# taintpro98/rnd-semantic-segmentation

Hardware: AMD Instinct MI355X
Metric: train images/sec at 769x769 bf16 (DeepLabV2-ResNet101 + ASPP) (higher is better)
Workload: dtype bf16; 1 GPU; train_src.py DeepLabV2-R101 bf16, 769x769 synthetic Cityscapes crops, batch 8 per GPU, 1xMI355X; global_batch=8, parallelism=dp1, weights=formula (synthetic), hip_graph_replay=False

## Files before the change

### rnd_semantic_segmentation_amd/csrc/igemm_common.h

```cpp
#pragma once
#include "mi_common.h"

namespace {

__device__ __attribute__((aligned(256))) uint32_t g_zero_page[64];

struct IgemmParams {
    const __bf16* A;
    const __bf16* Wp;
    void* out;
    const float* scale;
    const float* bias;
    const __bf16* res;
    const __bf16* msk;
    uint16_t* mask_out;
    int M, N, Ca, T;
    int Ho, Wo, Ha, Wa;
    int ksz, stride, pad, dil, mode;
    int flags, zgw;
    float alpha;
    int m_tiles, n_tiles;
    int korder;
    float* stats;
    const float* pilot;
};

__device__ __forceinline__ float igemm_row16_sum(float v) {
    v += __builtin_bit_cast(float, __builtin_amdgcn_update_dpp(0, __builtin_bit_cast(int, v), 0xB1, 0xF, 0xF, true));
    v += __builtin_bit_cast(float, __builtin_amdgcn_update_dpp(0, __builtin_bit_cast(int, v), 0x4E, 0xF, 0xF, true));
    v += __builtin_bit_cast(float, __builtin_amdgcn_update_dpp(0, __builtin_bit_cast(int, v), 0x141, 0xF, 0xF, true));
    v += __builtin_bit_cast(float, __builtin_amdgcn_update_dpp(0, __builtin_bit_cast(int, v), 0x140, 0xF, 0xF, true));
    return v;
}

__device__ __forceinline__ void glds16(const char* gsrc, char* lds_wave_base) {
    __builtin_amdgcn_global_load_lds((const __attribute__((address_space(1))) void*)gsrc,
                                     (__attribute__((address_space(3))) void*)lds_wave_base, 16, 0, 0);
}
__device__ __forceinline__ void glds16_nt(const char* gsrc, char* lds_wave_base) {
    __builtin_amdgcn_global_load_lds((const __attribute__((address_space(1))) void*)gsrc,
                                     (__attribute__((address_space(3))) void*)lds_wave_base, 16, 0, 2);
}

__device__ __forceinline__ void blds16(__amdgpu_buffer_rsrc_t rsrc, unsigned voffset, unsigned soffset, char* lds_wave_base) {
    __builtin_amdgcn_raw_ptr_buffer_load_lds(rsrc, (__attribute__((address_space(3))) void*)lds_wave_base, 16, voffset, soffset, 0, 0);
}


template <int MT, int EPI, bool WANT_RES = true>
__device__ __forceinline__ void igemm_fetch_epilogue(const IgemmParams& p, int m0, int n0, int wm, int wn, int frow, int fq, bf16x8 (&pres)[MT][2],
                                                     unsigned (&pbits)[MT], const int* mrow = nullptr) {
    const int flags = (EPI >= 0 ? EPI : p.flags) & (WANT_RES ? ~0 : ~MI_EPI_RESIDUAL);
    const int nbp = n0 + wn * 64 + 8 * fq;
#pragma unroll
    for (int j = 0; j < MT; ++j) {
        const int m = mrow ? (mrow[j] < 0 ? p.M : mrow[j]) : m0 + wm * (MT * 16) + j * 16 + frow;
        const long o0 = (long)(m < p.M ? m : 0) * p.N + (nbp < p.N ? nbp : 0);
        const long o1 = (long)(m < p.M ? m : 0) * p.N + (nbp + 32 < p.N ? nbp + 32 : 0);
        if (flags & MI_EPI_RESIDUAL) {
            pres[j][0] = *reinterpret_cast<const bf16x8*>(p.res + o0);
            pres[j][1] = *reinterpret_cast<const bf16x8*>(p.res + o1);
        }
        if (flags & MI_EPI_BITMASK) {
            const uint8_t* mb = reinterpret_cast<const uint8_t*>(p.msk);
            pbits[j] = (unsigned)mb[o0 >> 3] | ((unsigned)mb[o1 >> 3] << 8);
        }
    }
}

template <int MT, int EPI, bool STAGED = false>
__device__ __forceinline__ void igemm_epilogue(const IgemmParams& p, f32x4 (&acc)[4][MT], int m0, int n0, int wm, int wn, int frow, int fq,
                                               bf16x8 (&pres)[MT][2], unsigned (&pbits)[MT], char* stage = nullptr, bool mask_lds = false,
                                               const int* mrow = nullptr) {
    const int flags = EPI >= 0 ? EPI : p.flags;
    constexpr bool STATS = EPI >= 0 && (EPI & MI_EPI_STATS) != 0;
    float st0[STATS ? 16 : 1], st1[STATS ? 16 : 1];
    const int nb = n0 + wn * 64 + 8 * fq;
    f32x4 esc[4], ebi[4];
    if (flags & MI_EPI_SCALE_BIAS) {
#pragma unroll
        for (int i = 0; i < 4; ++i) {
            const int ni = nb + 32 * (i >> 1) + 4 * (i & 1);
            const int n = (ni < p.N) ? ni : 0;
            esc[i] = *reinterpret_cast<const f32x4*>(p.scale + n);
            ebi[i] = *reinterpret_cast<const f32x4*>(p.bias + n);
        }
    }
    f32x4 epil[4];
    if constexpr (STATS) {
#pragma unroll
        for (int i = 0; i < 4; ++i) {
            const int ni = nb + 32 * (i >> 1) + 4 * (i & 1);
            epil[i] = *reinterpret_cast<const f32x4*>(p.pilot + ((ni < p.N) ? ni : 0));
        }
#pragma unroll
        for (int k = 0; k < 16; ++k) st0[k] = st1[k] = 0.f;
#pragma unroll
        for (int i = 0; i < 4; ++i) asm volatile("" ::"v"(epil[i]));
    }
    if (flags & MI_EPI_SCALE_BIAS) {
#pragma unroll
        for (int i = 0; i < 4; ++i) asm volatile("" ::"v"(esc[i]), "v"(ebi[i]));
    }
    if (flags & MI_EPI_RESIDUAL) {
#pragma unroll
        for (int j = 0; j < MT; ++j) asm volatile("" ::"v"(pres[j][0]), "v"(pres[j][1]));
    }
    if (flags & MI_EPI_BITMASK) {
#pragma unroll
        for (int j = 0; j < MT; ++j) asm volatile("" ::"v"(pbits[j]));
    }
#pragma unroll
    for (int j = 0; j < MT; ++j) {
        const int m = mrow ? (mrow[j] < 0 ? p.M : mrow[j]) : m0 + wm * (MT * 16) + j * 16 + frow;
        if (m >= p.M) continue;
        const long o = (long)m * p.N + nb;
        f32x4 v[4];
#pragma unroll
        for (int i = 0; i < 4; ++i) v[i] = acc[i][j];
        if (flags & MI_EPI_SCALE_BIAS) {
#pragma unroll
            for (int i = 0; i < 4; ++i) v[i] = v[i] * esc[i] + ebi[i];
        }
        if (flags & MI_EPI_RESIDUAL) {
#pragma unroll
            for (int h = 0; h < 2; ++h) {
                if (nb + 32 * h < p.N) {
                    const bf16x8 r = pres[j][h];
#pragma unroll
                    for (int e = 0; e < 8; ++e) v[2 * h + (e >> 2)][e & 3] += (float)r[e];
                }
            }
        }
        if (flags & MI_EPI_RELU) {
            if (flags & MI_EPI_LEAKY) {
#pragma unroll
                for (int i = 0; i < 4; ++i)
#pragma unroll
                    for (int e = 0; e < 4; ++e) v[i][e] = v[i][e] > 0.f ? v[i][e] : p.alpha * v[i][e];
            } else {
#pragma unroll
                for (int i = 0; i < 4; ++i)
#pragma unroll
                    for (int e = 0; e < 4; ++e) asm("v_max_f32 %0, 0, %1" : "=v"(v[i][e]) : "v"(v[i][e]));
            }
        }
        if (flags & MI_EPI_MASK) {
#pragma unroll
            for (int h = 0; h < 2; ++h) {
                if (nb + 32 * h < p.N) {
                    const bf16x8 k = *reinterpret_cast<const bf16x8*>(p.msk + o + 32 * h);
#pragma unroll
                    for (int e = 0; e < 8; ++e)
                        v[2 * h + (e >> 2)][e & 3] = ((float)k[e] > 0.f) ? v[2 * h + (e >> 2)][e & 3] : 0.f;
                }
            }
        }
        if (flags & MI_EPI_BITMASK) {
            const float neg = (flags & MI_EPI_LEAKY) ? p.alpha : 0.f;
#pragma unroll
            for (int h = 0; h < 2; ++h) {
                if (nb + 32 * h < p.N) {
                    const unsigned bits = (pbits[j] >> (8 * h)) & 0xffu;
                    if (flags & MI_EPI_LEAKY) {
#pragma unroll
                        for (int c = 0; c < 8; ++c) v[2 * h + (c >> 2)][c & 3] = ((bits >> c) & 1u) ? v[2 * h + (c >> 2)][c & 3] : neg * v[2 * h + (c >> 2)][c & 3];
                    } else {
#pragma unroll
                        for (int c = 0; c < 8; ++c) {
                            const unsigned keep = (unsigned)__builtin_amdgcn_sbfe((int)bits, c, 1);
                            v[2 * h + (c >> 2)][c & 3] = __uint_as_float(__float_as_uint(v[2 * h + (c >> 2)][c & 3]) & keep);
                        }
                    }
                }
            }
        }
        if (flags & MI_EPI_WRITE_MASK) {
#pragma unroll
            for (int h = 0; h < 2; ++h) {
                if (nb + 32 * h < p.N) {
                    unsigned bits = 0;
                    if ((flags & MI_EPI_RELU) && !(flags & MI_EPI_LEAKY)) {
#pragma unroll
                        for (int c = 7; c >= 0; --c) bits = __builtin_amdgcn_alignbit(bits, 0u - __float_as_uint(v[2 * h + (c >> 2)][c & 3]), 31);
                    } else {
#pragma unroll
                        for (int c = 0; c < 8; ++c) bits |= (v[2 * h + (c >> 2)][c & 3] > 0.f ? 1u : 0u) << c;
                    }
                    if (STAGED && mask_lds)
                        reinterpret_cast<uint8_t*>(stage)[MT * 32 * 256 + (wm * (MT * 16) + j * 16 + frow) * 16 + wn * 8 + h * 4 + fq] = (uint8_t)bits;
                    else
                        reinterpret_cast<uint8_t*>(p.mask_out)[(o + 32 * h) >> 3] = (uint8_t)bits;
                }
            }
        }
        if (flags & MI_EPI_ZSPLIT) {
#pragma unroll
            for (int i = 0; i < 4; ++i) {
                const int n = nb + 32 * (i >> 1) + 4 * (i & 1);
                if (n < p.N) {
                    const int g = n / p.zgw, nn = n - g * p.zgw;
                    *reinterpret_cast<f32x4*>(reinterpret_cast<float*>(p.out) + ((long)g * p.M + m) * p.zgw + nn) = v[i];
                }
            }
        } else if (flags & MI_EPI_OUT_F32) {
#pragma unroll
            for (int i = 0; i < 4; ++i) {
                const int n = nb + 32 * (i >> 1) + 4 * (i & 1);
                if (n < p.N) *reinterpret_cast<f32x4*>(reinterpret_cast<float*>(p.out) + (long)m * p.N + n) = v[i];
            }
        } else {
#pragma unroll
            for (int h = 0; h < 2; ++h) {
                if (nb + 32 * h < p.N) {
                    bf16x8 hv;
#pragma unroll
                    for (int e = 0; e < 8; ++e) hv[e] = (__bf16)v[2 * h + (e >> 2)][e & 3];
                    if constexpr (STATS) {
#pragma unroll
                        for (int e = 0; e < 8; ++e) {
                            const float d = (float)hv[e] - epil[2 * h + (e >> 2)][e & 3];
                            st0[8 * h + e] += d;
                            st1[8 * h + e] += d * d;
                        }
                    }
                    if (STAGED) {
                        const int row = wm * (MT * 16) + j * 16 + frow;
                        *reinterpret_cast<bf16x8*>(stage + row * 256 + (((wn * 8 + h * 4 + fq) ^ (row & 15)) << 4)) = hv;
                    } else {
                        *reinterpret_cast<bf16x8*>(reinterpret_cast<__bf16*>(p.out) + o + 32 * h) = hv;
                    }
                }
            }
        }
    }
    if constexpr (STATS) {
#pragma unroll
        for (int k = 0; k < 16; ++k) st0[k] = igemm_row16_sum(st0[k]), st1[k] = igemm_row16_sum(st1[k]);
        if (frow == 0) {
            const long rt = (m0 + wm * (MT * 16)) / (MT * 16);
            float* dst = p.stats + rt * 2 * (long)p.N;
#pragma unroll
            for (int h = 0; h < 2; ++h) {
                if (nb + 32 * h < p.N) {
#pragma unroll
                    for (int q = 0; q < 2; ++q) {
                        *reinterpret_cast<f32x4*>(dst + nb + 32 * h + 4 * q) = f32x4{st0[8 * h + 4 * q], st0[8 * h + 4 * q + 1], st0[8 * h + 4 * q + 2], st0[8 * h + 4 * q + 3]};
                        *reinterpret_cast<f32x4*>(dst + p.N + nb + 32 * h + 4 * q) = f32x4{st1[8 * h + 4 * q], st1[8 * h + 4 * q + 1], st1[8 * h + 4 * q + 2], st1[8 * h + 4 * q + 3]};
                    }
                }
            }
        }
    }
}

template <int MT>
__device__ __forceinline__ void igemm_residual_to_lds(const IgemmParams& p, int m0, int n0, int wave, int lane, const char* zero, char* stage) {
    const int prow = lane >> 4, pch = lane & 15;
#pragma unroll
    for (int i = 0; i < 2 * MT; ++i) {
        const int q = wave + 4 * i;
        const int row = 4 * q + prow, m = m0 + row;
        const int n = n0 + ((pch ^ (row & 15)) << 3);
        const char* src = (m < p.M && n < p.N) ? reinterpret_cast<const char*>(p.res + (long)m * p.N + n) : zero;
        glds16(src, stage + q * 1024);
    }
}

template <int MT>
__device__ __forceinline__ void igemm_residual_from_lds(const char* stage, int wm, int wn, int frow, int fq, bf16x8 (&pres)[MT][2]) {
#pragma unroll
    for (int j = 0; j < MT; ++j) {
        const int row = wm * (MT * 16) + j * 16 + frow;
#pragma unroll
        for (int h = 0; h < 2; ++h) pres[j][h] = *reinterpret_cast<const bf16x8*>(stage + row * 256 + (((wn * 8 + h * 4 + fq) ^ (row & 15)) << 4));
    }
}

template <int MT>
__device__ __forceinline__ void igemm_mask_to_lds(const IgemmParams& p, int m0, int n0, int tid, char* stage) {
    if (tid < MT * 32) {
        const int m = m0 + tid;
        u32x4 v = {0u, 0u, 0u, 0u};
        if (m < p.M) v = *reinterpret_cast<const u32x4*>(reinterpret_cast<const uint8_t*>(p.msk) + (((long)m * p.N + n0) >> 3));
        *reinterpret_cast<u32x4*>(stage + MT * 32 * 256 + tid * 16) = v;
    }
}

template <int MT>
__device__ __forceinline__ void igemm_mask_from_lds(const char* stage, int wm, int wn, int frow, int fq, unsigned (&pbits)[MT]) {
    const uint8_t* img = reinterpret_cast<const uint8_t*>(stage) + MT * 32 * 256;
#pragma unroll
    for (int j = 0; j < MT; ++j) {
        const int base = (wm * (MT * 16) + j * 16 + frow) * 16 + wn * 8 + fq;
        pbits[j] = (unsigned)img[base] | ((unsigned)img[base + 4] << 8);
    }
}

template <int MT>
__device__ __forceinline__ void igemm_store_mask_staged(const IgemmParams& p, int m0, int n0, int tid, const char* stage) {
    if (tid < MT * 32) {
        const int m = m0 + tid;
        if (m < p.M)
            *reinterpret_cast<u32x4*>(reinterpret_cast<uint8_t*>(p.mask_out) + (((long)m * p.N + n0) >> 3)) =
                *reinterpret_cast<const u32x4*>(stage + MT * 32 * 256 + tid * 16);
    }
}

template <int MT>
__device__ __forceinline__ void igemm_store_staged(const IgemmParams& p, int m0, int n0, int tid, const char* stage) {
    const int c = tid & 15, r_in = tid >> 4;
    const int n = n0 + c * 8;
    if (n >= p.N) return;
#pragma unroll
    for (int it = 0; it < 2 * MT; ++it) {
        const int row = it * 16 + r_in, m = m0 + row;
        if (m < p.M) {
            __builtin_nontemporal_store(*reinterpret_cast<const u32x4*>(stage + row * 256 + ((c ^ (row & 15)) << 4)),
                                        reinterpret_cast<u32x4*>(reinterpret_cast<__bf16*>(p.out) + (long)m * p.N + n));
        }
    }
}

}
```

### rnd_semantic_segmentation_amd/csrc/igemm_nt.hip

```cpp
#include "igemm_common.h"
#include <stdlib.h>

namespace {

template <int MT, int BKT = 64, int NWN = 2> struct Geo {
    static constexpr int NW = 2 * NWN;
    static constexpr int BM = 32 * MT, BNT = 64 * NWN;
    static constexpr int ROWB = BKT * 2;
    static constexpr int RPP = 1024 / ROWB;
    static constexpr int CPR = ROWB / 16;
    static constexpr int PA = BM / RPP;
    static constexpr int NPA = (PA + NW - 1) / NW;
    static constexpr int NPW = BNT / RPP / NW;
    static constexpr int ATILE_BYTES = BM * ROWB;
    static constexpr int WTILE_BYTES = BNT * ROWB;
    static constexpr int STAGE_BYTES = ATILE_BYTES + WTILE_BYTES;
    static constexpr int LDS_BYTES = 2 * STAGE_BYTES;
    static constexpr int OCC = NWN == 4 ? 1 : (BKT == 64 ? 2 : (MT <= 4 ? 4 : 3));
};

__device__ __forceinline__ bool tap_src(const IgemmParams& p, int ho, int wo, int ky, int kx, int& ha, int& wa) {
    const bool fwd = p.mode == MI_GATHER_FWD;
    const int fh = ho * p.stride + ky * p.dil - p.pad, fw = wo * p.stride + kx * p.dil - p.pad;
    const int nh = ho + p.pad - ky * p.dil, nw = wo + p.pad - kx * p.dil;
    const int qh = nh / p.stride, qw = nw / p.stride;
    const bool dg_ok = (nh >= 0) & (nw >= 0) & (qh * p.stride == nh) & (qw * p.stride == nw);
    ha = fwd ? fh : qh;
    wa = fwd ? fw : qw;
    return (fwd | dg_ok) & ((unsigned)ha < (unsigned)p.Ha) & ((unsigned)wa < (unsigned)p.Wa);
}

template <int MT, bool UNIT, bool PREF, int BKT, int EPI, int NWN, bool STG = false>
__global__ __launch_bounds__((Geo<MT, BKT, NWN>::NW * 64), (Geo<MT, BKT, NWN>::OCC)) void igemm_nt_kernel(IgemmParams p) {
    static_assert(!STG || (EPI >= 0 && !PREF && NWN == 2 && BKT == 64 && !(EPI & (MI_EPI_OUT_F32 | MI_EPI_ZSPLIT))), "staged epilogue: hot bf16 sets only");
    using G = Geo<MT, BKT, NWN>;
    constexpr int BM = G::BM, BN = G::BNT, ATILE_BYTES = G::ATILE_BYTES, STAGE_BYTES = G::STAGE_BYTES;
    constexpr int ROWB = G::ROWB, RPP = G::RPP, CPR = G::CPR, NPA = G::NPA, NPW = G::NPW, NW = G::NW;
    static_assert(BM % RPP == 0 && BN % (RPP * NW) == 0, "tiles must split into whole DMA pieces");
    extern __shared__ __attribute__((aligned(16))) char smem[];
    const int tid = threadIdx.x, lane = tid & 63;
    const int wave = __builtin_amdgcn_readfirstlane(tid >> 6);
    const int nwg = p.m_tiles * p.n_tiles;
    const int tile = mi_xcd_remap(blockIdx.x, nwg);
    const int mt = tile / p.n_tiles, nt = tile - mt * p.n_tiles;
    const int m0 = mt * BM, n0 = nt * BN;

    const int prow = lane / CPR, pch = lane % CPR;
    const char* zero = reinterpret_cast<const char*>(g_zero_page);
    int a_img[NPA], a_ho[NPA], a_wo[NPA];
    const char* a_base[NPA];
    unsigned a_mask[NPA];
    const int HoWo = p.Ho * p.Wo;
    const int a_chunk = (pch ^ (BKT == 64 ? (prow & 7) : ((prow >> 2) & 3))) * 16;
    constexpr int PA_BASE = G::PA / NW, PA_REM = G::PA % NW;
    const int a_first = wave * PA_BASE + (wave < PA_REM ? wave : PA_REM);
    const int a_count = PA_BASE + (wave < PA_REM ? 1 : 0);
    const int sgn = (p.mode == MI_GATHER_FWD) ? 1 : -1;
    const bool pointwise = UNIT && p.T == 1 && p.pad == 0;
    int cb_ = 0, cho = 0, cwo = 0;
#pragma unroll
    for (int i = 0; i < NPA; ++i) {
        const int m = m0 + (a_first + i) * RPP + prow;
        const bool ok = (m < p.M) & (i < a_count);
        if (pointwise) {
            a_base[i] = reinterpret_cast<const char*>(p.A + (long)(ok ? m : 0) * p.Ca) + a_chunk;
            a_mask[i] = ok ? 1u : 0u;
            a_ho[i] = a_wo[i] = 0;
            a_img[i] = -1;
            continue;
        }
        if (!UNIT || i == 0) {
            const int mm = ok ? m : 0;
            cb_ = mm / HoWo;
            const int rem = mm - cb_ * HoWo;
            cho = rem / p.Wo;
            cwo = rem - cho * p.Wo;
        } else {
            cwo += RPP;
            while (cwo >= p.Wo) {
                cwo -= p.Wo;
                ++cho;
            }
            while (cho >= p.Ho) {
                cho -= p.Ho;
                ++cb_;
            }
        }
        const int b = cb_, ho = cho, wo = cwo;
        a_ho[i] = ho;
        a_wo[i] = wo;
        a_img[i] = ok ? b * p.Ha * p.Wa : -1;
        if (UNIT) {
            const int h0 = ho - sgn * p.pad, w0 = wo - sgn * p.pad;
            a_base[i] = reinterpret_cast<const char*>(p.A + ((long)b * p.Ha * p.Wa + (long)h0 * p.Wa + w0) * p.Ca) + a_chunk;
            unsigned rb = 0, cb = 0;
#pragma unroll
            for (int kq = 0; kq < 3; ++kq) {
                const bool live = kq < p.ksz;
                rb |= (unsigned)(live & ((unsigned)(h0 + sgn * kq * p.dil) < (unsigned)p.Ha)) << kq;
                cb |= (unsigned)(live & ((unsigned)(w0 + sgn * kq * p.dil) < (unsigned)p.Wa)) << kq;
            }
            unsigned msk;
            if (p.ksz == 1) msk = rb & cb & 1u;
            else msk = ((rb & 1u) ? cb : 0u) | ((rb & 2u) ? cb << 3 : 0u) | ((rb & 4u) ? cb << 6 : 0u);
            a_mask[i] = ok ? msk : 0u;
        }
    }
    int w_row[NPW], w_chunk[NPW];
    const char* w_base[NPW];
#pragma unroll
    for (int i = 0; i < NPW; ++i) {
        const int rl = (wave * NPW + i) * RPP + prow;
        w_row[i] = n0 + rl;
        w_chunk[i] = (pch ^ (BKT == 64 ? ((rl & 3) | (((rl >> 3) & 1) << 2)) : ((rl >> 3) & 3))) * 16;
        w_base[i] = reinterpret_cast<const char*>(p.Wp + (long)(w_row[i] < p.N ? w_row[i] : 0) * p.Ca) + w_chunk[i];
    }

    const int cpt = p.Ca / BKT;
    const int nk = p.T * cpt;
    int ld_t = 0, ld_cc = 0;
    const char* a_ptr[NPA];
    const char* w_ptr[NPW];
    int a_inc[NPA], w_inc[NPW];
    const long w_tap_bytes = (long)p.N * p.Ca * 2;

    auto set_tap = [&](int t) __attribute__((always_inline)) {
        const int ky = t / p.ksz, kx = t - ky * p.ksz;
        if (UNIT) {
            const long toff = (long)sgn * ((long)ky * p.dil * p.Wa + (long)kx * p.dil) * p.Ca * 2;
#pragma unroll
            for (int i = 0; i < NPA; ++i) {
                const bool ok = (a_mask[i] >> t) & 1u;
                a_ptr[i] = ok ? a_base[i] + toff : zero;
                a_inc[i] = ok ? ROWB : 0;
            }
        } else {
#pragma unroll
            for (int i = 0; i < NPA; ++i) {
                int ha = 0, wa = 0;
                const bool ok = tap_src(p, a_ho[i], a_wo[i], ky, kx, ha, wa) && a_img[i] >= 0;
                const char* ptr = reinterpret_cast<const char*>(p.A + ((long)((ok ? a_img[i] : 0) + (ok ? ha : 0) * p.Wa + (ok ? wa : 0))) * p.Ca) + a_chunk;
                a_ptr[i] = ok ? ptr : zero;
                a_inc[i] = ok ? ROWB : 0;
            }
        }
        const long woff = (long)t * w_tap_bytes;
#pragma unroll
        for (int i = 0; i < NPW; ++i) {
            const bool ok = w_row[i] < p.N;
            w_ptr[i] = ok ? w_base[i] + woff : zero;
            w_inc[i] = ok ? ROWB : 0;
        }
    };
    set_tap(0);

    auto stage = [&](int buf) {
        char* sa = smem + buf * STAGE_BYTES + a_first * 1024;
        char* sb = smem + buf * STAGE_BYTES + ATILE_BYTES + wave * (NPW * 1024);
#pragma unroll
        for (int i = 0; i < NPA; ++i) {
            if (PA_REM == 0 || i < a_count) glds16(a_ptr[i], sa + i * 1024);
            a_ptr[i] += a_inc[i];
        }
#pragma unroll
        for (int i = 0; i < NPW; ++i) {
            glds16(w_ptr[i], sb + i * 1024);
            w_ptr[i] += w_inc[i];
        }
        if (++ld_cc == cpt) {
            ld_cc = 0;
            ++ld_t;
            if (ld_t < p.T) set_tap(ld_t);
        }
    };

    const int wm = wave & 1, wn = wave >> 1;
    f32x4 acc[4][MT];
#pragma unroll
    for (int i = 0; i < 4; ++i)
#pragma unroll
        for (int j = 0; j < MT; ++j) acc[i][j] = f32x4{0.f, 0.f, 0.f, 0.f};

    const int frow = lane & 15, fq = lane >> 4;
    const int wrow0 = wn * 64 + 8 * (frow >> 2) + (frow & 3);
    const int flags = EPI >= 0 ? EPI : p.flags;
    bf16x8 pres[MT][2];
    unsigned pbits[MT];
    if (PREF) igemm_fetch_epilogue<MT, EPI>(p, m0, n0, wm, wn, frow, fq, pres, pbits);
    auto compute = [&](int buf) {
        const char* sa = smem + buf * STAGE_BYTES;
        const char* sb = sa + ATILE_BYTES;
#pragma unroll
        for (int kk = 0; kk < BKT / 32; ++kk) {
            const int sw = BKT == 64 ? (((kk * 4 + fq) ^ (frow & 7)) << 4) : ((fq ^ ((frow >> 2) & 3)) << 4);
            bf16x8 wf[4], af[MT];
#pragma unroll
            for (int i = 0; i < 4; ++i) wf[i] = *reinterpret_cast<const bf16x8*>(sb + (wrow0 + 32 * (i >> 1) + 4 * (i & 1)) * ROWB + sw);
#pragma unroll
            for (int j = 0; j < MT; ++j) af[j] = *reinterpret_cast<const bf16x8*>(sa + (wm * (MT * 16) + j * 16 + frow) * ROWB + sw);
#pragma unroll
            for (int i = 0; i < 4; ++i)
#pragma unroll
                for (int j = 0; j < MT; ++j) acc[i][j] = __builtin_amdgcn_mfma_f32_16x16x32_bf16(wf[i], af[j], acc[i][j], 0, 0, 0);
        }
    };

    stage(0);
    asm volatile("s_waitcnt vmcnt(0)" ::: "memory");
    __syncthreads();
    for (int kt = 0; kt < nk; ++kt) {
        const int cur = kt & 1;
        if (kt + 1 < nk) stage(cur ^ 1);
        compute(cur);
        asm volatile("s_waitcnt vmcnt(0)" ::: "memory");
        __syncthreads();
    }

    if (EPI < 0 && (p.flags & (1 << 30))) {
#pragma unroll
        for (int i = 0; i < 4; ++i)
#pragma unroll
            for (int j = 0; j < MT; ++j) asm volatile("" ::"v"(acc[i][j]));
        return;
    }
    if constexpr (STG) {
        constexpr bool RES = (EPI & MI_EPI_RESIDUAL) != 0, BITS_IN = (EPI & MI_EPI_BITMASK) != 0, BITS_OUT = (EPI & MI_EPI_WRITE_MASK) != 0;
        const bool mask_lds = (p.N & 127) == 0;
        if (RES) igemm_residual_to_lds<MT>(p, m0, n0, wave, lane, zero, smem);
        if (BITS_IN) {
            if (mask_lds) igemm_mask_to_lds<MT>(p, m0, n0, tid, smem);
            else igemm_fetch_epilogue<MT, EPI, false>(p, m0, n0, wm, wn, frow, fq, pres, pbits);
        }
        if (RES || BITS_IN) {
            asm volatile("s_waitcnt vmcnt(0)" ::: "memory");
            __syncthreads();
            if (RES) igemm_residual_from_lds<MT>(smem, wm, wn, frow, fq, pres);
            if (BITS_IN && mask_lds) igemm_mask_from_lds<MT>(smem, wm, wn, frow, fq, pbits);
        }
        igemm_epilogue<MT, EPI, true>(p, acc, m0, n0, wm, wn, frow, fq, pres, pbits, smem, mask_lds);
        __syncthreads();
        igemm_store_staged<MT>(p, m0, n0, tid, smem);
        if (BITS_OUT && mask_lds) igemm_store_mask_staged<MT>(p, m0, n0, tid, smem);
        return;
    }
    if (!PREF) igemm_fetch_epilogue<MT, EPI>(p, m0, n0, wm, wn, frow, fq, pres, pbits);
    igemm_epilogue<MT, EPI>(p, acc, m0, n0, wm, wn, frow, fq, pres, pbits);
}

inline bool staged_on() { return mi_sw().igemm_staged != 0; }

template <int MT, bool UNIT, bool PREF, int BKT, int EPI, int NWN, bool STG = false>
void launch_one(dim3 grid, hipStream_t stream, const IgemmParams& p) {
    static std::atomic<uint64_t> attr_done{0};
    auto kern = igemm_nt_kernel<MT, UNIT, PREF, BKT, EPI, NWN, STG>;
    constexpr int lds = Geo<MT, BKT, NWN>::LDS_BYTES;
    mi_allow_dynamic_lds((const void*)kern, lds, attr_done);
    hipLaunchKernelGGL(kern, grid, dim3(Geo<MT, BKT, NWN>::NW * 64), lds, stream, p);
}

template <int MT, bool UNIT, bool PREF, int BKT, int NWN>
void launch_variant(dim3 grid, hipStream_t stream, const IgemmParams& p, int epi, bool staged) {
    if constexpr (UNIT) {
        if constexpr (!PREF && NWN == 2 && BKT == 64) {
            if (staged) {
                if (epi == 71) return launch_one<MT, UNIT, PREF, BKT, 71, NWN, true>(grid, stream, p);
                if (epi == 130) return launch_one<MT, UNIT, PREF, BKT, 130, NWN, true>(grid, stream, p);
            }
        }
        if constexpr (!PREF) {
            if (epi == 69) return launch_one<MT, UNIT, PREF, BKT, 69, NWN>(grid, stream, p);
            if (epi == 128) return launch_one<MT, UNIT, PREF, BKT, 128, NWN>(grid, stream, p);
        }
        if (epi == 71) return launch_one<MT, UNIT, PREF, BKT, 71, NWN>(grid, stream, p);
        if (epi == 130) return launch_one<MT, UNIT, PREF, BKT, 130, NWN>(grid, stream, p);
    }
    if constexpr (!PREF && NWN == 2) {
        if (epi == MI_EPI_STATS) return launch_one<MT, UNIT, PREF, BKT, MI_EPI_STATS, NWN>(grid, stream, p);
    }
    launch_one<MT, UNIT, PREF, BKT, -1, NWN>(grid, stream, p);
}

bool pp_by_rule(int B, int Ha, int Wa, int Ca, int Ho, int Wo, int N, int ksize, int stride, int flags) {
    const int pp_on = mi_sw().igemm_pp;
    const int min_k = mi_sw().igemm_pp_mink;
    const long M = (long)B * Ho * Wo;
    return pp_on && stride == 1 && Ha == Ho && Wa == Wo && !(flags & (MI_EPI_RESIDUAL | MI_EPI_MASK | MI_EPI_LEAKY)) && (long)ksize * ksize * Ca >= min_k &&
           Ca % 32 == 0 && M >= 320 * 64 && N >= 256;
}

}

extern "C" int mi_conv_gemm_pp(const void* a, const void* wp, void* out, int B, int Ha, int Wa, int Ca, int Ho, int Wo, int N, int ksize,
                               int stride, int pad, int dil, int gather_mode, const float* scale, const float* bias, const void* res,
                               const void* msk, void* mask_out, int flags, int zgw, float alpha, int mtg, void* stream);

#define PLAN_REQUIRE(cond, ...)                      \
    do {                                             \
        if (!(cond)) {                               \
            snprintf(why, PLAN_WHY_LEN, __VA_ARGS__); \
            return MI_EINVAL;                        \
        }                                            \
    } while (0)
constexpr int PLAN_WHY_LEN = 256;
static int conv_plan(int B, int Ha, int Wa, int Ca, int Ho, int Wo, int N, int ksize, int stride, int pad, int dil, int flags, int pp_mtg, MiConvPlan* pl,
                     char* why) {
    PLAN_REQUIRE(B > 0 && Ha > 0 && Wa > 0 && Ho > 0 && Wo > 0 && N > 0, "mi_conv_gemm: non-positive dimension");
    PLAN_REQUIRE(Ca > 0 && Ca % 32 == 0, "mi_conv_gemm: Ca=%d must be a multiple of 32", Ca);
    PLAN_REQUIRE(ksize == 1 || ksize == 3, "mi_conv_gemm: ksize=%d (1 or 3)", ksize);
    PLAN_REQUIRE(stride >= 1 && dil >= 1 && pad >= 0, "mi_conv_gemm: bad stride/dil/pad");
    const long M = (long)B * Ho * Wo;
    PLAN_REQUIRE(M < (1L << 31) && (long)B * Ha * Wa < (1L << 31), "mi_conv_gemm: pixel count overflows int32");
    const bool same = stride == 1 && Ha == Ho && Wa == Wo;
    const long lim = (1L << 31) - (1L << 20);
    const long a_bytes = (long)B * Ha * Wa * Ca * 2 + 2L * ((long)(ksize - 1) * dil + pad) * (Wa + 1) * Ca * 2, w_bytes = (long)ksize * ksize * N * Ca * 2;
    const bool fits32 = a_bytes < lim && w_bytes < lim;
    const bool fits32_rule = (long)B * Ha * Wa * Ca * 2 + 64L * (Wa + 1) * Ca * 2 < lim;
    const bool pp_only = Ca % 64 != 0;
    bool pp = pp_mtg >= 0;
    if (pp_mtg < 0) {
        if (pp_only) {
            PLAN_REQUIRE(same && !(flags & (MI_EPI_RESIDUAL | MI_EPI_MASK | MI_EPI_LEAKY)),
                       "mi_conv_gemm: Ca=%d is not a multiple of 64: stride-1, same-size launches without residual / mask / LeakyReLU only", Ca);
            PLAN_REQUIRE(fits32, "mi_conv_gemm: Ca=%d is not a multiple of 64 and the operands exceed the 2 GiB the 32-channel main loop addresses", Ca);
            pp = true;
        } else {
            pp = fits32 && fits32_rule && pp_by_rule(B, Ha, Wa, Ca, Ho, Wo, N, ksize, stride, flags);
        }
    }
    MiConvPlan& r = *pl;
    r = MiConvPlan{};
    if (pp) {
        PLAN_REQUIRE(same, "mi_conv_gemm_pp: stride-1, same-size convolutions only");
        PLAN_REQUIRE(fits32, "mi_conv_gemm_pp: operand larger than 2 GiB");
        int mtg = pp_mtg;
        if (mtg != 8 && mtg != 10) {
            auto rounds = [&](int bm) { return (((M + bm - 1) / bm) * ((N + 255) / 256) + 255) / 256; };
            mtg = rounds(320) < rounds(256) ? 10 : (rounds(256) < rounds(320) ? 8 : (((M + 319) / 320) * 320 <= ((M + 255) / 256) * 256 ? 10 : 8));
        }
        r.kernel = MI_CPLAN_PP;
        r.mt = mtg;
        r.bn = 256;
        r.unit = 1;
        r.korder = ksize > 1 ? mi_sw().pp_korder : 0;
        r.epi = (flags == 69 || flags == 128 || flags == 0 || flags == 1 || flags == 48 || flags == MI_EPI_STATS) ? flags : -1;
        r.m_tiles = (int)((M + 32 * mtg - 1) / (32 * mtg));
        r.n_tiles = (N + 255) / 256;
        r.slots = 256;
        r.rounds = (int)(((long)r.m_tiles * r.n_tiles + 255) / 256);
        return MI_OK;
    }
    const bool unit = same && ksize * ksize <= 9;
    const int force_mt = mi_sw().igemm_mt, force_bn = mi_sw().igemm_bn, pref_on = mi_sw().igemm_pref;
    auto cost = [&](int bm, int bn) {
        const int per_cu = bn == 256 ? 1 : 2;
        const long tiles = ((M + bm - 1) / bm) * ((N + bn - 1) / bn);
        const long rounds = (tiles + 256 * per_cu - 1) / (256 * per_cu);
        const double t_l2 = (bm + bn) * 128.0 / 47.6e3, t_mfma = bm * (double)bn * 128.0 / 9.77e6;
        return rounds * per_cu * ((t_l2 > t_mfma ? t_l2 : t_mfma) + 0.2 * (t_l2 > t_mfma ? t_mfma : t_l2));
    };
#ifdef MI_EXPERIMENTS
    const bool wide_ok = unit && N % 256 == 0 && !(flags & MI_EPI_ZSPLIT) && force_bn == 256;
#else
    const bool wide_ok = false;
    (void)force_bn;
#endif
    int mt_sel = 4, bn = 128;
    double best = cost(128, 128);
    for (int mt = 5; mt <= 6; ++mt)
        if (cost(32 * mt, 128) < best * 0.999) best = cost(32 * mt, 128), mt_sel = mt;
    if (force_mt >= 4 && force_mt <= 6) mt_sel = force_mt, best = cost(32 * mt_sel, 128);
    if (wide_ok) {
        int wmt = 0;
        double wbest = force_bn == 256 ? 1e30 : best;
        for (int mt = 4; mt <= 6; ++mt)
            if ((force_mt == 0 || force_mt == mt) && cost(32 * mt, 256) < wbest * 0.999) wbest = cost(32 * mt, 256), wmt = mt;
        if (wmt) mt_sel = wmt, bn = 256;
    }
    const bool hot_set = flags == 71 || flags == 130;
    const bool pref = bn == 128 && pref_on && unit && (flags & MI_EPI_RESIDUAL) && N % 16 == 0 && !(staged_on() && hot_set);
    if (!unit) mt_sel = 4;
    if (pref && mt_sel == 6) mt_sel = 5;
    const int bm = mt_sel * 32;
    r.kernel = MI_CPLAN_NT;
    r.mt = mt_sel;
    r.bn = bn;
    r.unit = unit;
    r.pref = pref && bn == 128;
    r.staged = unit && !pref && bn == 128 && staged_on() && hot_set;
    if (unit && (hot_set || (!pref && (flags == 69 || flags == 128)))) r.epi = flags;
    else if (!pref && bn == 128 && flags == MI_EPI_STATS) r.epi = MI_EPI_STATS;
    else r.epi = -1;
    r.m_tiles = (int)((M + bm - 1) / bm);
    r.n_tiles = (N + bn - 1) / bn;
    r.slots = bn == 256 ? 256 : 512;
    r.rounds = (int)(((long)r.m_tiles * r.n_tiles + r.slots - 1) / r.slots);
    return MI_OK;
}
#undef PLAN_REQUIRE

int mi_conv_plan(int B, int Ha, int Wa, int Ca, int Ho, int Wo, int N, int ksize, int stride, int pad, int dil, int flags, int pp_mtg, MiConvPlan* pl) {
    char why[PLAN_WHY_LEN];
    const int rc = conv_plan(B, Ha, Wa, Ca, Ho, Wo, N, ksize, stride, pad, dil, flags, pp_mtg, pl, why);
    return rc == MI_OK ? MI_OK : mi_set_error(rc, "%s", why);
}

extern "C" int mi_conv_gemm_plan(int B, int Ha, int Wa, int Ca, int Ho, int Wo, int N, int ksize, int stride, int pad, int dil, int flags, int pp_mtg, int* plan) {
    MI_REQUIRE(plan, "mi_conv_gemm_plan: null plan");
    MI_REQUIRE(pp_mtg == -1 || pp_mtg == 0 || pp_mtg == 8 || pp_mtg == 10, "mi_conv_gemm_plan: pp_mtg=%d (-1: mi_conv_gemm, 0 | 8 | 10: mi_conv_gemm_pp)", pp_mtg);
    MiConvPlan r;
    const int rc = mi_conv_plan(B, Ha, Wa, Ca, Ho, Wo, N, ksize, stride, pad, dil, flags, pp_mtg, &r);
    if (rc != MI_OK) return rc;
    const int v[MI_CPLAN_LEN] = {r.kernel, r.mt, r.unit, r.pref, r.staged, r.epi, r.korder, r.m_tiles, r.n_tiles, r.rounds, r.slots};
    for (int k = 0; k < MI_CPLAN_LEN; ++k) plan[k] = v[k];
    return MI_OK;
}

extern "C" int mi_conv_gemm_route(int B, int Ha, int Wa, int Ca, int Ho, int Wo, int N, int ksize, int stride, int flags) {
    MiConvPlan r;
    char why[PLAN_WHY_LEN];
    if (conv_plan(B, Ha, Wa, Ca, Ho, Wo, N, ksize, stride, 32 - (ksize == 3 ? 2 : 0), 1, flags, -1, &r, why) != MI_OK) return 0;
    return r.kernel == MI_CPLAN_PP;
}

extern "C" int mi_conv_gemm(const void* a, const void* wp, void* out, int B, int Ha, int Wa, int Ca, int Ho, int Wo, int N,
                            int ksize, int stride, int pad, int dil, int gather_mode, const float* scale, const float* bias,
                            const void* res, const void* msk, void* mask_out, int flags, int zgw, float alpha, void* stream) {
    return mi_conv_gemm_impl(a, wp, out, B, Ha, Wa, Ca, Ho, Wo, N, ksize, stride, pad, dil, gather_mode, scale, bias, res, msk, mask_out, flags, zgw, alpha,
                             stream, nullptr);
}

extern "C" size_t mi_conv_gemm_stats_workspace(long M, int N) {
    const long rows = (M + 63) / 64 + 2;
    return ((size_t)rows * 2 * (size_t)N + mi_bn_reduce_tmp_floats((int)rows, N)) * sizeof(float);
}

extern "C" int mi_conv_gemm_stats(const void* a, const void* wp, void* out, int B, int Ha, int Wa, int Ca, int Ho, int Wo, int N, int ksize, int stride,
                                  int pad, int dil, const float* pilot, float* sums, void* workspace, size_t workspace_bytes, const float* gamma,
                                  const float* beta, float* running_mean, float* running_var, long long* num_batches_tracked, float momentum, float eps,
                                  float* out4, void* stream) {
    MI_REQUIRE(pilot && sums && workspace && mi_aligned16(pilot) && mi_aligned16(workspace), "mi_conv_gemm_stats: null or unaligned statistics operand");
    MI_REQUIRE(B > 0 && Ho > 0 && Wo > 0 && N > 0 && N % 8 == 0, "mi_conv_gemm_stats: N=%d", N);
    const long M = (long)B * Ho * Wo;
    MI_REQUIRE(workspace_bytes >= mi_conv_gemm_stats_workspace(M, N), "mi_conv_gemm_stats: workspace of %zu bytes, need %zu", workspace_bytes,
               mi_conv_gemm_stats_workspace(M, N));
    MI_REQUIRE((gamma == nullptr) == (out4 == nullptr), "mi_conv_gemm_stats: gamma and out4 go together (finalize in the same call) or are both NULL");
    MiConvStats st{(float*)workspace, pilot, 0};
    const int rc = mi_conv_gemm_impl(a, wp, out, B, Ha, Wa, Ca, Ho, Wo, N, ksize, stride, pad, dil, MI_GATHER_FWD, nullptr, nullptr, nullptr, nullptr, nullptr,
                                     MI_EPI_STATS, 0, 0.f, stream, &st);
    if (rc != MI_OK) return rc;
    float* tmp = (float*)workspace + ((M + 63) / 64 + 2) * 2 * (long)N;
    const MiBnFinal fin{pilot, (double)M, gamma, beta, running_mean, running_var, num_batches_tracked, momentum, eps, out4};
    return mi_bn_reduce_partials((const float*)workspace, st.nparts, N, tmp, sums, sums + N, gamma ? &fin : nullptr, stream);
}

int mi_conv_gemm_impl(const void* a, const void* wp, void* out, int B, int Ha, int Wa, int Ca, int Ho, int Wo, int N, int ksize, int stride, int pad,
                      int dil, int gather_mode, const float* scale, const float* bias, const void* res, const void* msk, void* mask_out, int flags,
                      int zgw, float alpha, void* stream, MiConvStats* st) {
    MI_REQUIRE(a && wp && out, "mi_conv_gemm: null operand");
    MI_REQUIRE(((flags & MI_EPI_STATS) != 0) == (st != nullptr) && (!st || flags == MI_EPI_STATS), "mi_conv_gemm: MI_EPI_STATS comes alone, through mi_conv_gemm_stats");
    MI_REQUIRE(B > 0 && Ha > 0 && Wa > 0 && Ho > 0 && Wo > 0 && N > 0, "mi_conv_gemm: non-positive dimension");
    MI_REQUIRE(Ca > 0 && Ca % 32 == 0, "mi_conv_gemm: Ca=%d must be a multiple of 32", Ca);
    MI_REQUIRE(Ca % 64 == 0 || (stride == 1 && Ha == Ho && Wa == Wo && !(flags & (MI_EPI_RESIDUAL | MI_EPI_MASK | MI_EPI_LEAKY))),
               "mi_conv_gemm: Ca=%d is not a multiple of 64: stride-1, same-size launches without residual / mask / LeakyReLU only", Ca);
    MI_REQUIRE(N % 8 == 0, "mi_conv_gemm: N=%d must be a multiple of 8", N);
    MI_REQUIRE(ksize == 1 || ksize == 3, "mi_conv_gemm: ksize=%d (1 or 3)", ksize);
    MI_REQUIRE(stride >= 1 && dil >= 1 && pad >= 0, "mi_conv_gemm: bad stride/dil/pad");
    MI_REQUIRE(gather_mode == MI_GATHER_FWD || gather_mode == MI_GATHER_DGRAD, "mi_conv_gemm: gather_mode");
    MI_REQUIRE(mi_aligned16(a) && mi_aligned16(wp) && mi_aligned16(out), "mi_conv_gemm: operands must be 16-byte aligned");
    MI_REQUIRE(!(flags & MI_EPI_SCALE_BIAS) || (scale && bias && mi_aligned16(scale) && mi_aligned16(bias)), "mi_conv_gemm: scale/bias");
    MI_REQUIRE(!(flags & MI_EPI_RESIDUAL) || (res && mi_aligned16(res)), "mi_conv_gemm: residual");
    MI_REQUIRE(!(flags & MI_EPI_MASK) || (msk && mi_aligned16(msk)), "mi_conv_gemm: mask");
    MI_REQUIRE(!(flags & MI_EPI_BITMASK) || (msk && N % 16 == 0 && !(flags & MI_EPI_MASK)), "mi_conv_gemm: bit mask needs N %% 16 == 0");
    MI_REQUIRE(!(flags & MI_EPI_WRITE_MASK) || (mask_out && N % 16 == 0), "mi_conv_gemm: mask_out needs N %% 16 == 0");
    MI_REQUIRE(!(flags & MI_EPI_BITMASK) || N % 128 != 0 || mi_aligned16(msk), "mi_conv_gemm: the packed sign bits must be 16-byte aligned");
    MI_REQUIRE(!(flags & MI_EPI_WRITE_MASK) || N % 128 != 0 || mi_aligned16(mask_out), "mi_conv_gemm: mask_out must be 16-byte aligned");
    MI_REQUIRE(!(flags & MI_EPI_ZSPLIT) || (zgw > 0 && zgw % 4 == 0 && N % zgw == 0), "mi_conv_gemm: zgw");
    const long M = (long)B * Ho * Wo;
    MI_REQUIRE(M < (1L << 31) && (long)B * Ha * Wa < (1L << 31), "mi_conv_gemm: pixel count overflows int32");
    if (gather_mode == MI_GATHER_FWD) {
        MI_REQUIRE((Ho - 1) * stride - pad < Ha && (Wo - 1) * stride - pad < Wa, "mi_conv_gemm: output larger than the input supports");
    }
    MiConvPlan pl;
    {
        const int rc = mi_conv_plan(B, Ha, Wa, Ca, Ho, Wo, N, ksize, stride, pad, dil, flags, -1, &pl);
        if (rc != MI_OK) return rc;
    }
    if (pl.kernel == MI_CPLAN_PP)
        return mi_conv_gemm_pp_impl(a, wp, out, B, Ha, Wa, Ca, Ho, Wo, N, ksize, stride, pad, dil, gather_mode, scale, bias, res, msk, mask_out, flags, zgw,
                                    alpha, 0, stream, st);
    IgemmParams p;
    p.korder = 0;
    p.stats = st ? st->partial : nullptr;
    p.pilot = st ? st->pilot : nullptr;
    p.A = (const __bf16*)a;
    p.Wp = (const __bf16*)wp;
    p.out = out;
    p.scale = scale;
    p.bias = bias;
    p.res = (const __bf16*)res;
    p.msk = (const __bf16*)msk;
    p.mask_out = (uint16_t*)mask_out;
    p.M = (int)M;
    p.N = N;
    p.Ca = Ca;
    p.T = ksize * ksize;
    p.Ho = Ho;
    p.Wo = Wo;
    p.Ha = Ha;
    p.Wa = Wa;
    p.ksz = ksize;
    p.stride = stride;
    p.pad = pad;
    p.dil = dil;
    p.mode = gather_mode;
    p.flags = flags;
    p.zgw = zgw > 0 ? zgw : 4;
    p.alpha = alpha;
    p.m_tiles = pl.m_tiles;
    p.n_tiles = pl.n_tiles;
    const dim3 grid(p.m_tiles * p.n_tiles);
    if (st) st->nparts = 2 * p.m_tiles;
    const hipStream_t sq = (hipStream_t)stream;
    const int epi = pl.epi;
    const bool stg = pl.staged != 0;
    if (!pl.unit)
        launch_variant<4, false, false, 64, 2>(grid, sq, p, epi, stg);
#ifdef MI_EXPERIMENTS
    else if (pl.bn == 256 && pl.mt == 6)
        launch_variant<6, true, false, 64, 4>(grid, sq, p, epi, stg);
    else if (pl.bn == 256 && pl.mt == 5)
        launch_variant<5, true, false, 64, 4>(grid, sq, p, epi, stg);
    else if (pl.bn == 256)
        launch_variant<4, true, false, 64, 4>(grid, sq, p, epi, stg);
#endif
    else if (pl.pref && pl.mt == 5)
        launch_variant<5, true, true, 64, 2>(grid, sq, p, epi, stg);
    else if (pl.pref)
        launch_variant<4, true, true, 64, 2>(grid, sq, p, epi, stg);
    else if (pl.mt == 6)
        launch_variant<6, true, false, 64, 2>(grid, sq, p, epi, stg);
    else if (pl.mt == 5)
        launch_variant<5, true, false, 64, 2>(grid, sq, p, epi, stg);
    else
        launch_variant<4, true, false, 64, 2>(grid, sq, p, epi, stg);
    MI_CHECK_LAUNCH("mi_conv_gemm");
    return MI_OK;
}
```

Baseline: 293.2 images/s.

## Overlap residual and mask epilogue loads with the final K-loop iterations

For the staged-epilogue implicit-GEMM kernel with residual, the last K iterations are peeled. The residual tile's global-to-LDS loads and the mask loads are issued before the final compute step, with part of the residual held in registers and written to LDS afterwards. This hides epilogue fetch latency behind the last MFMA work instead of paying it serially after the loop. The default NT_STG_LOOP=2 enables only this residual-overlap path; an optional 4-slot BK=32 ring pipeline is added behind a compile-time switch. The cost is extra registers for the held residual and more fragile vmcnt bookkeeping.

```diff
diff --git a/rnd_semantic_segmentation_amd/csrc/igemm_common.h b/rnd_semantic_segmentation_amd/csrc/igemm_common.h
--- a/rnd_semantic_segmentation_amd/csrc/igemm_common.h
+++ b/rnd_semantic_segmentation_amd/csrc/igemm_common.h
@@ -42,6 +42,12 @@
                                      (__attribute__((address_space(3))) void*)lds_wave_base, 16, 0, 2);
 }
 
+template <int N>
+__device__ __forceinline__ void igemm_wait_vm() {
+    static_assert(N >= 0 && N < 64, "vmcnt is a 6-bit count");
+    asm volatile("s_waitcnt vmcnt(%0)" ::"n"(N) : "memory");
+}
+
 __device__ __forceinline__ void blds16(__amdgpu_buffer_rsrc_t rsrc, unsigned voffset, unsigned soffset, char* lds_wave_base) {
     __builtin_amdgcn_raw_ptr_buffer_load_lds(rsrc, (__attribute__((address_space(3))) void*)lds_wave_base, 16, voffset, soffset, 0, 0);
 }
@@ -254,11 +260,11 @@
     }
 }
 
-template <int MT>
+template <int MT, int I0 = 0, int I1 = 2 * MT>
 __device__ __forceinline__ void igemm_residual_to_lds(const IgemmParams& p, int m0, int n0, int wave, int lane, const char* zero, char* stage) {
     const int prow = lane >> 4, pch = lane & 15;
 #pragma unroll
-    for (int i = 0; i < 2 * MT; ++i) {
+    for (int i = I0; i < I1; ++i) {
         const int q = wave + 4 * i;
         const int row = 4 * q + prow, m = m0 + row;
         const int n = n0 + ((pch ^ (row & 15)) << 3);
@@ -267,6 +273,25 @@
     }
 }
 
+template <int MT, int I0, int I1>
+__device__ __forceinline__ void igemm_residual_load(const IgemmParams& p, int m0, int n0, int wave, int lane, u32x4 (&r)[I1 > I0 ? I1 - I0 : 1]) {
+    const int prow = lane >> 4, pch = lane & 15;
+#pragma unroll
+    for (int i = I0; i < I1; ++i) {
+        const int row = 4 * (wave + 4 * i) + prow, m = m0 + row;
+        const int n = n0 + ((pch ^ (row & 15)) << 3);
+        const bool ok = m < p.M && n < p.N;
+        const u32x4 v = *reinterpret_cast<const u32x4*>(p.res + (ok ? (long)m * p.N + n : 0));
+        r[i - I0] = ok ? v : u32x4{0u, 0u, 0u, 0u};
+    }
+}
+
+template <int MT, int I0, int I1>
+__device__ __forceinline__ void igemm_residual_put(int wave, int lane, const u32x4 (&r)[I1 > I0 ? I1 - I0 : 1], char* stage) {
+#pragma unroll
+    for (int i = I0; i < I1; ++i) *reinterpret_cast<u32x4*>(stage + (wave + 4 * i) * 1024 + lane * 16) = r[i - I0];
+}
+
 template <int MT>
 __device__ __forceinline__ void igemm_residual_from_lds(const char* stage, int wm, int wn, int frow, int fq, bf16x8 (&pres)[MT][2]) {
 #pragma unroll
@@ -278,13 +303,21 @@
 }
 
 template <int MT>
+__device__ __forceinline__ u32x4 igemm_mask_load(const IgemmParams& p, int m0, int n0, int tid) {
+    const int m = m0 + tid;
+    u32x4 v = {0u, 0u, 0u, 0u};
+    if (tid < MT * 32 && m < p.M) v = *reinterpret_cast<const u32x4*>(reinterpret_cast<const uint8_t*>(p.msk) + (((long)m * p.N + n0) >> 3));
+    return v;
+}
+
+template <int MT>
+__device__ __forceinline__ void igemm_mask_put(int tid, u32x4 v, char* stage) {
+    if (tid < MT * 32) *reinterpret_cast<u32x4*>(stage + MT * 32 * 256 + tid * 16) = v;
+}
+
+template <int MT>
 __device__ __forceinline__ void igemm_mask_to_lds(const IgemmParams& p, int m0, int n0, int tid, char* stage) {
-    if (tid < MT * 32) {
-        const int m = m0 + tid;
-        u32x4 v = {0u, 0u, 0u, 0u};
-        if (m < p.M) v = *reinterpret_cast<const u32x4*>(reinterpret_cast<const uint8_t*>(p.msk) + (((long)m * p.N + n0) >> 3));
-        *reinterpret_cast<u32x4*>(stage + MT * 32 * 256 + tid * 16) = v;
-    }
+    igemm_mask_put<MT>(tid, igemm_mask_load<MT>(p, m0, n0, tid), stage);
 }
 
 template <int MT>
diff --git a/rnd_semantic_segmentation_amd/csrc/igemm_nt.hip b/rnd_semantic_segmentation_amd/csrc/igemm_nt.hip
--- a/rnd_semantic_segmentation_amd/csrc/igemm_nt.hip
+++ b/rnd_semantic_segmentation_amd/csrc/igemm_nt.hip
@@ -1,5 +1,6 @@
 #include "igemm_common.h"
 #include <stdlib.h>
+#include <type_traits>
 
 namespace {
 
@@ -30,10 +31,20 @@
     return (fwd | dg_ok) & ((unsigned)ha < (unsigned)p.Ha) & ((unsigned)wa < (unsigned)p.Wa);
 }
 
+#if defined(MI_EXPERIMENTS) && defined(MI_NT_STG_LOOP)
+constexpr int NT_STG_LOOP = MI_NT_STG_LOOP;
+#else
+constexpr int NT_STG_LOOP = 2;
+#endif
+static_assert(NT_STG_LOOP >= 0 && NT_STG_LOOP <= 3, "MI_NT_STG_LOOP: 0..3");
+
 template <int MT, bool UNIT, bool PREF, int BKT, int EPI, int NWN, bool STG = false>
 __global__ __launch_bounds__((Geo<MT, BKT, NWN>::NW * 64), (Geo<MT, BKT, NWN>::OCC)) void igemm_nt_kernel(IgemmParams p) {
     static_assert(!STG || (EPI >= 0 && !PREF && NWN == 2 && BKT == 64 && !(EPI & (MI_EPI_OUT_F32 | MI_EPI_ZSPLIT))), "staged epilogue: hot bf16 sets only");
-    using G = Geo<MT, BKT, NWN>;
+    constexpr bool RING = STG && (NT_STG_LOOP & 1) != 0, RESU = STG && (NT_STG_LOOP & 2) != 0 && (EPI & MI_EPI_RESIDUAL) != 0;
+    constexpr int BKS = RING ? 32 : BKT;
+    using G = Geo<MT, BKS, NWN>;
+    static_assert(!RING || 4 * G::STAGE_BYTES == Geo<MT, BKT, NWN>::LDS_BYTES, "the slab ring lives in the double buffer's LDS");
     constexpr int BM = G::BM, BN = G::BNT, ATILE_BYTES = G::ATILE_BYTES, STAGE_BYTES = G::STAGE_BYTES;
     constexpr int ROWB = G::ROWB, RPP = G::RPP, CPR = G::CPR, NPA = G::NPA, NPW = G::NPW, NW = G::NW;
     static_assert(BM % RPP == 0 && BN % (RPP * NW) == 0, "tiles must split into whole DMA pieces");
@@ -51,7 +62,7 @@
     const char* a_base[NPA];
     unsigned a_mask[NPA];
     const int HoWo = p.Ho * p.Wo;
-    const int a_chunk = (pch ^ (BKT == 64 ? (prow & 7) : ((prow >> 2) & 3))) * 16;
+    const int a_chunk = (pch ^ (BKS == 64 ? (prow & 7) : ((prow >> 2) & 3))) * 16;
     constexpr int PA_BASE = G::PA / NW, PA_REM = G::PA % NW;
     const int a_first = wave * PA_BASE + (wave < PA_REM ? wave : PA_REM);
     const int a_count = PA_BASE + (wave < PA_REM ? 1 : 0);
@@ -112,11 +123,11 @@
     for (int i = 0; i < NPW; ++i) {
         const int rl = (wave * NPW + i) * RPP + prow;
         w_row[i] = n0 + rl;
-        w_chunk[i] = (pch ^ (BKT == 64 ? ((rl & 3) | (((rl >> 3) & 1) << 2)) : ((rl >> 3) & 3))) * 16;
+        w_chunk[i] = (pch ^ (BKS == 64 ? ((rl & 3) | (((rl >> 3) & 1) << 2)) : ((rl >> 3) & 3))) * 16;
         w_base[i] = reinterpret_cast<const char*>(p.Wp + (long)(w_row[i] < p.N ? w_row[i] : 0) * p.Ca) + w_chunk[i];
     }
 
-    const int cpt = p.Ca / BKT;
+    const int cpt = p.Ca / BKS;
     const int nk = p.T * cpt;
     int ld_t = 0, ld_cc = 0;
     const char* a_ptr[NPA];
@@ -191,8 +202,8 @@
         const char* sa = smem + buf * STAGE_BYTES;
         const char* sb = sa + ATILE_BYTES;
 #pragma unroll
-        for (int kk = 0; kk < BKT / 32; ++kk) {
-            const int sw = BKT == 64 ? (((kk * 4 + fq) ^ (frow & 7)) << 4) : ((fq ^ ((frow >> 2) & 3)) << 4);
+        for (int kk = 0; kk < BKS / 32; ++kk) {
+            const int sw = BKS == 64 ? (((kk * 4 + fq) ^ (frow & 7)) << 4) : ((fq ^ ((frow >> 2) & 3)) << 4);
             bf16x8 wf[4], af[MT];
 #pragma unroll
             for (int i = 0; i < 4; ++i) wf[i] = *reinterpret_cast<const bf16x8*>(sb + (wrow0 + 32 * (i >> 1) + 4 * (i & 1)) * ROWB + sw);
@@ -205,15 +216,102 @@
         }
     };
 
-    stage(0);
-    asm volatile("s_waitcnt vmcnt(0)" ::: "memory");
-    __syncthreads();
-    for (int kt = 0; kt < nk; ++kt) {
-        const int cur = kt & 1;
-        if (kt + 1 < nk) stage(cur ^ 1);
-        compute(cur);
+    constexpr bool MASK_IN = STG && (EPI >= 0) && (EPI & MI_EPI_BITMASK) != 0;
+    const bool mask_lds = (p.N & 127) == 0;
+    u32x4 mbits = {0u, 0u, 0u, 0u};
+    if constexpr (RING) {
+        constexpr int SKP = STAGE_BYTES / 1024, NPR = 8 * MT;
+        constexpr int I0 = (SKP / 4 < 2 * MT ? SKP / 4 : 2 * MT), I1 = (2 * SKP / 4 < 2 * MT ? 2 * SKP / 4 : 2 * MT), I2 = 2 * MT;
+        constexpr int R0 = RESU ? I0 : 0, R1 = RESU ? I1 - I0 : 0;
+        static_assert(NPR <= 3 * SKP && BM * 272 <= 3 * STAGE_BYTES, "the residual and mask images must end below the last slab's slot");
+        constexpr int PS_HI = NPA + NPW, PS_LO = PS_HI - (PA_REM != 0 ? 1 : 0);
+        auto wait_landed = [&](auto s_, auto e_) __attribute__((always_inline)) {
+            constexpr int S = decltype(s_)::value, E = decltype(e_)::value;
+            if (PA_REM != 0 && wave >= PA_REM) igemm_wait_vm<S * PS_LO + E>();
+            else igemm_wait_vm<S * PS_HI + E>();
+        };
+        using std::integral_constant;
+        const int ns = nk;
+        int ld_slot = (4 - ns) & 3, cp_slot = ld_slot;
+        for (int s = 0; s < 4 && s < ns; ++s, ld_slot = (ld_slot + 1) & 3) stage(ld_slot);
+        auto step = [&](int s, auto last_) __attribute__((always_inline)) {
+            constexpr bool LAST = decltype(last_)::value;
+            if (s == 0) {
+                if (ns >= 4) wait_landed(integral_constant<int, 3>{}, integral_constant<int, 0>{});
+                else if (ns == 3) wait_landed(integral_constant<int, 2>{}, integral_constant<int, 0>{});
+                else if (ns == 2) wait_landed(integral_constant<int, 1>{}, integral_constant<int, 0>{});
+                else igemm_wait_vm<0>();
+            } else if (LAST) {
+                wait_landed(integral_constant<int, 0>{}, integral_constant<int, R0 + R1>{});
+            } else if (s == ns - 2) {
+                wait_landed(integral_constant<int, 1>{}, integral_constant<int, R0>{});
+            } else {
+                wait_landed(integral_constant<int, 2>{}, integral_constant<int, 0>{});
+            }
+            __builtin_amdgcn_s_barrier();
+            if (!LAST && s >= 1 && s + 3 < ns) {
+                stage(ld_slot);
+                ld_slot = (ld_slot + 1) & 3;
+            }
+            if constexpr (RESU) {
+                if (s == (ns > 3 ? ns - 3 : 0)) igemm_residual_to_lds<MT, 0, I0>(p, m0, n0, wave, lane, zero, smem);
+                if (s == (ns > 2 ? ns - 2 : 0)) igemm_residual_to_lds<MT, I0, I1>(p, m0, n0, wave, lane, zero, smem);
+                if constexpr (LAST) {
+                    igemm_residual_to_lds<MT, I1, I2>(p, m0, n0, wave, lane, zero, smem);
+                    if (MASK_IN && mask_lds) mbits = igemm_mask_load<MT>(p, m0, n0, tid);
+                }
+            }
+            compute(cp_slot);
+            cp_slot = (cp_slot + 1) & 3;
+            asm volatile("s_waitcnt lgkmcnt(0)" ::: "memory");
+            __builtin_amdgcn_sched_barrier(0);
+        };
+        for (int s = 0; s + 1 < ns; ++s) step(s, std::false_type{});
+        step(ns - 1, std::true_type{});
+    } else if constexpr (RESU) {
+        constexpr int IH = (STAGE_BYTES / 4096 < 2 * MT ? STAGE_BYTES / 4096 : 2 * MT);
+        constexpr int NOV = 2 * MT - IH;
+        static_assert(STAGE_BYTES % 4096 == 0, "a stage must hold whole rounds of the four waves' residual pieces");
+        constexpr int PS_HI = NPA + NPW, PS_LO = PS_HI - (PA_REM != 0 ? 1 : 0);
+        u32x4 rov[NOV > 0 ? NOV : 1];
+        int slot = nk & 1;
+        stage(slot);
+        if (nk > 1) stage(slot ^ 1);
+        for (int kt = 0; kt + 1 < nk; ++kt) {
+            if (kt == 0) {
+                if (PA_REM != 0 && wave >= PA_REM) igemm_wait_vm<PS_LO>();
+                else igemm_wait_vm<PS_HI>();
+            } else {
+                igemm_wait_vm<0>();
+            }
+            __builtin_amdgcn_s_barrier();
+            if (kt >= 1) stage(slot ^ 1);
+            compute(slot);
+            slot ^= 1;
+            asm volatile("s_waitcnt lgkmcnt(0)" ::: "memory");
+            __builtin_amdgcn_sched_barrier(0);
+        }
+        igemm_wait_vm<0>();
+        __builtin_amdgcn_s_barrier();
+        igemm_residual_to_lds<MT, 0, IH>(p, m0, n0, wave, lane, zero, smem);
+        igemm_residual_load<MT, IH, 2 * MT>(p, m0, n0, wave, lane, rov);
+        if (MASK_IN && mask_lds) mbits = igemm_mask_load<MT>(p, m0, n0, tid);
+        compute(1);
+        asm volatile("s_waitcnt lgkmcnt(0)" ::: "memory");
+        __builtin_amdgcn_sched_barrier(0);
+        __builtin_amdgcn_s_barrier();
+        igemm_residual_put<MT, IH, 2 * MT>(wave, lane, rov, smem);
+    } else {
+        stage(0);
         asm volatile("s_waitcnt vmcnt(0)" ::: "memory");
         __syncthreads();
+        for (int kt = 0; kt < nk; ++kt) {
+            const int cur = kt & 1;
+            if (kt + 1 < nk) stage(cur ^ 1);
+            compute(cur);
+            asm volatile("s_waitcnt vmcnt(0)" ::: "memory");
+            __syncthreads();
+        }
     }
 
     if (EPI < 0 && (p.flags & (1 << 30))) {
@@ -225,10 +323,10 @@
     }
     if constexpr (STG) {
         constexpr bool RES = (EPI & MI_EPI_RESIDUAL) != 0, BITS_IN = (EPI & MI_EPI_BITMASK) != 0, BITS_OUT = (EPI & MI_EPI_WRITE_MASK) != 0;
-        const bool mask_lds = (p.N & 127) == 0;
-        if (RES) igemm_residual_to_lds<MT>(p, m0, n0, wave, lane, zero, smem);
+        if (RES && !RESU) igemm_residual_to_lds<MT>(p, m0, n0, wave, lane, zero, smem);
         if (BITS_IN) {
-            if (mask_lds) igemm_mask_to_lds<MT>(p, m0, n0, tid, smem);
+            if (mask_lds && RESU) igemm_mask_put<MT>(tid, mbits, smem);
+            else if (mask_lds) igemm_mask_to_lds<MT>(p, m0, n0, tid, smem);
             else igemm_fetch_epilogue<MT, EPI, false>(p, m0, n0, wm, wn, frow, fq, pres, pbits);
         }
         if (RES || BITS_IN) {
```

Result: no change. 295.3 images/s (median of 6 runs) (+0.7%).
